# NUStatBioinfo/DegNorm

Hardware: AMD Instinct MI355X
Metric: genes/sec (20k genes x 10 samples, 5 iters) (higher is better)
Workload: dtype f64

## Files before the change

### degnorm_amd/csrc/dn_kernels.hpp

```cpp
#pragma once
#include <hip/hip_runtime.h>
#include <stddef.h>
#include <stdint.h>
#include <type_traits>
#include "dn_reduce.hpp"
#include "dn_dpp_ops.hpp"

#ifdef DN_MARKS
#define DN_MARK(name) asm volatile("; DN_MARK " name)
#else
#define DN_MARK(name)
#endif

namespace dn {

constexpr int TRACE_LEN = 48;
constexpr int MAX_BINS = 64;
constexpr int P_MAX = 64;
constexpr int P_WIDE_MAX = 256;

enum { EXIT_LOW_COV = 0, EXIT_ZERO_SAMPLE = 1, EXIT_MEDIAN = 2, EXIT_NO_LOOP = 3,
       EXIT_REFINED = 4, EXIT_REFINE_FALLBACK = 5, EXIT_NOT_FOUND_FALLBACK = 6 };
enum { LOOP_NATURAL = 0, LOOP_PERFECT = 1, LOOP_VALUE_ERROR = 2, LOOP_ZERO_ROWSUM = 3, LOOP_MIN_BINS = 4,
       LOOP_NOT_ENTERED = 5 };
// ... 656 lines not shown
    y = lds_row_dot<P>(Gr, uv);
    theta = wave_allsum(ul * y);
    return capped ? maxs + 1 : (steps < maxs ? steps + 1 : maxs);
}

constexpr double WARM_START_MIN_COMPONENT = 1e-7;
template <int P, bool DPP = (P <= 16)> struct Solver;
template <int P> struct Solver<P, true> {
    EigStateD<P> st;
    __device__ __forceinline__ double iterate_of_row() const { return st.vl; }
    static __device__ __forceinline__ int row_of_lane() { return lane_id() & 15; }
    static __device__ __forceinline__ double bcast_component(double t, int i) { return bcast_lane<P>(t, i); }
    __device__ __forceinline__ void cold(double tr, double (&u)[P]) { (void) u; eig_state_cold<P>(st, tr); }
    __device__ __forceinline__ void start_from(unsigned long long rows, double (&u)[P])
    {
        (void) u;
        const double u0 = 1.0 / sqrt((double) __builtin_popcountll(rows));
        st.vl = ((rows >> (lane_id() & 15)) & 1ull) ? u0 : 0.0;
        st.k0 = 0; st.rho2 = 1.0; st.q = 1.0; st.age = 0;
    }
    __device__ __forceinline__ void no_shift()
    {
        st.mu = 0.0;
    }
    __device__ __forceinline__ double shift() const { return st.mu; }
    __device__ __forceinline__ double scale() const { return st.sc; }
    static constexpr bool SHIFTED = true;
    static constexpr bool SQUARE = true;
    template <bool SQ = false>
    __device__ __forceinline__ int run(const double *tot, int zslot, double (&u)[P], double &theta, bool exact, int maxs, bool cold = false,
                                       const double *sq = nullptr)
    {
        return top_eig_dpp<P, false, SQ>(tot, zslot, u, theta, st, exact, cold, maxs, nullptr, sq);
    }
};
template <int P> struct Solver<P, false> {
    __device__ __forceinline__ void cold(double tr, double (&u)[P])
    {
        (void) tr;
        const double u0 = 1.0 / sqrt((double) P);
#pragma unroll
        for (int i = 0; i < P; i++) u[i] = u0;
    }
    __device__ __forceinline__ void start_from(unsigned long long rows, double (&u)[P])
    {
        const double u0 = 1.0 / sqrt((double) __builtin_popcountll(rows));
#pragma unroll
        for (int i = 0; i < P; i++) u[i] = ((rows >> i) & 1ull) ? u0 : 0.0;
    }
    __device__ __forceinline__ void no_shift() {}
    __device__ __forceinline__ double shift() const { return 0.0; }
    __device__ __forceinline__ double scale() const { return 1.0; }
    static constexpr bool SHIFTED = false;
    static constexpr bool SQUARE = false;
    template <bool SQ = false>
    __device__ __forceinline__ int run(const double *tot, int zslot, double (&u)[P], double &theta, bool exact, int maxs, bool cold = false,
                                       const double *sq = nullptr)
    { (void) zslot; (void) exact; (void) cold; (void) sq; return top_eig_rows<P>(tot, u, theta, maxs); }
};

__device__ __forceinline__ unsigned long long uniform_u64(unsigned long long x)
{
    const unsigned lo = __builtin_amdgcn_readfirstlane((unsigned) x), hi = __builtin_amdgcn_readfirstlane((unsigned) (x >> 32));
    return ((unsigned long long) hi << 32) | lo;
}

__device__ __forceinline__ unsigned long long gram_component(const double *tot, int seed, int nrows)
{
    const int lane = lane_id();
    unsigned long long comp = 1ull << seed, frontier = comp;
    while (frontier) {
        const int i = __builtin_ctzll(frontier);
        frontier &= frontier - 1ull;
        const int j = lane < nrows ? lane : 0;
        const int a = i > j ? i : j, b = i > j ? j : i;
        const bool link = lane < nrows && j != i && tot[a * (a + 1) / 2 + b] > 0.0;
        const unsigned long long fresh = uniform_u64(__ballot(link)) & ~comp;
        comp |= fresh;
        frontier |= fresh;
    }
    return comp;
}

template <int P>
__device__ __forceinline__ int solve_by_blocks(Solver<P> &solver, const double *tot, int zslot, double (&u)[P], double &theta,
                                               int maxs, int nrows = P)
{
    unsigned long long todo = nrows >= 64 ? ~0ull : ((1ull << nrows) - 1ull);
    const Solver<P> entry = solver;
    Solver<P> best = solver;
    double bu[P], bth = -1.0;
#pragma unroll
    for (int i = 0; i < P; i++) bu[i] = 0.0;
    int steps = 0;
    bool capped = false;
    while (todo) {
        const unsigned long long comp = gram_component(tot, __builtin_ctzll(todo), nrows);
        todo &= ~comp;
        Solver<P> s = entry;
        double uu[P], th = 0.0;
#pragma unroll
        for (int i = 0; i < P; i++) uu[i] = 0.0;
        s.start_from(comp, uu);
        const int r = s.run(tot, zslot, uu, th, true, maxs);
        steps += r < maxs ? r : maxs;
        capped = capped || r > maxs;
        if (th > bth) {
            bth = th;
            best = s;
#pragma unroll
            for (int i = 0; i < P; i++) bu[i] = uu[i];
        }
    }
    solver = best;
    solver.no_shift();
#pragma unroll
    for (int i = 0; i < P; i++) u[i] = bu[i];
    theta = bth > 0.0 ? bth : 0.0;
    return capped ? maxs + 1 : (steps < maxs ? steps : maxs);
}

typedef double gram_t;

template <int P, int LO, int CNT, typename T>
__device__ __forceinline__ void gram_add_range(T (&G)[CNT], const double (&a)[P])
{
    T b[P];
#pragma unroll
    for (int i = 0; i < P; i++) b[i] = (T) a[i];
#pragma unroll
    for (int i = 0; i < P; i++)
#pragma unroll
        for (int j = 0; j <= i; j++) {
            constexpr int dummy = 0; (void) dummy;
            const int idx = i * (i + 1) / 2 + j;
            if (idx >= LO && idx < LO + CNT) G[idx - LO] = fma(b[i], b[j], G[idx - LO]);
        }
}

template <int P, int LO, int CNT, typename T>
__device__ __forceinline__ void gram_set_range(T (&G)[CNT], const double (&a)[P])
{
    T b[P];
#pragma unroll
    for (int i = 0; i < P; i++) b[i] = (T) a[i];
#pragma unroll
    for (int i = 0; i < P; i++)
#pragma unroll
        for (int j = 0; j <= i; j++) {
            const int idx = i * (i + 1) / 2 + j;
            if (idx >= LO && idx < LO + CNT) G[idx - LO] = b[i] * b[j];
        }
}

template <int P, typename T>
__device__ __forceinline__ void gram_add(T (&G)[P * (P + 1) / 2], const double (&a)[P])
{
    T b[P];
#pragma unroll
    for (int i = 0; i < P; i++) b[i] = (T) a[i];
#pragma unroll
    for (int i = 0; i < P; i++)
#pragma unroll
        for (int j = 0; j <= i; j++) G[i * (i + 1) / 2 + j] = fma(b[i], b[j], G[i * (i + 1) / 2 + j]);
}

template <int P> __device__ __forceinline__ double vmax(const double (&v)[P])
{ double m = v[0];
#pragma unroll
  for (int i = 1; i < P; i++) m = v[i] > m ? v[i] : m; return m; }
template <int P> __device__ __forceinline__ double vmin(const double (&v)[P])
{ double m = v[0];
#pragma unroll
  for (int i = 1; i < P; i++) m = v[i] < m ? v[i] : m; return m; }

template <int P> __device__ __forceinline__ int fix_k(double (&K)[P])
{
    double mn = INFINITY;
#pragma unroll
    for (int i = 0; i < P; i++) { K[i] = fabs(K[i]); if (K[i] >= 1e-5 && K[i] < mn) mn = K[i]; }
    if (mn == INFINITY) return ST_EMPTY_MIN;
#pragma unroll
    for (int i = 0; i < P; i++) if (K[i] < 1e-5) K[i] = mn;
    return ST_OK;
}

template <int P> __device__ __forceinline__ double median_of(const double (&v)[P])
{
    double lo = 0.0, hi = 0.0;
#pragma unroll
    for (int i = 0; i < P; i++) {
        int less = 0, eq = 0;
#pragma unroll
        for (int j = 0; j < P; j++) { less += v[j] < v[i]; eq += v[j] == v[i]; }
        const int r_lo = (P - 1) / 2, r_hi = P / 2;
        if (less <= r_lo && r_lo < less + eq) lo = v[i];
        if (less <= r_hi && r_hi < less + eq) hi = v[i];
    }
    return 0.5 * (lo + hi);
}

template <int P>
struct GeneState {
    double sumF[P];
    double rho[P];
    double K[P];
    double us[P];
    double rho_fb[P];
    double sig0;
    double inv[P];
    double scl[P];
    double u[P];
    double theta;
    double sums[2 * P + 1];
    int32_t steps;
    int32_t status;
    int32_t max_steps;
#ifdef DN_STAMP
    long long stamp[8];
#else
    long long stamp[6];
#endif
};

#ifdef DN_P
__shared__ Smem<DN_P, DN_NT> g_sm_u[DN_UNITS];
__shared__ GeneState<DN_P> g_gs_u[DN_UNITS];
extern __shared__ __attribute__((aligned(16))) double g_lam[];
#define g_sm g_sm_u[DN_UNIT]
#define g_gs g_gs_u[DN_UNIT]
typedef const float __attribute__((address_space(1))) *gF_cptr;
typedef double __attribute__((address_space(1))) *gdouble_ptr;

template <int P>
__device__ __forceinline__ void col_update(const double (&f)[P], double (&a)[P], const double (&u)[P], const double (&ur)[P], double c)
{
    double s0 = 0.0, s1 = 0.0;
#pragma unroll
    for (int i = 0; i + 1 < P; i += 2) { s0 = fma(u[i], a[i], s0); s1 = fma(u[i + 1], a[i + 1], s1); }
    if (P & 1) s0 = fma(u[P - 1], a[P - 1], s0);
    const double s = s0 + s1;
#pragma unroll
    for (int i = 0; i < P; i++) {
        const double res = fma(ur[i], s, -f[i]);
        a[i] = fmax(fma(-c, res, a[i]), f[i]);
    }
}

template <int P>
__device__ __forceinline__ void col_update_lds(const float (&x)[P], const double *invp, double (&a)[P], const double *uv, double c)
{
    double s0 = 0.0, s1 = 0.0;
#pragma unroll
    for (int i = 0; i + 1 < P; i += 2) {
        const double2 u2 = *reinterpret_cast<const double2 *>(uv + i);
        s0 = fma(u2.x, a[i], s0); s1 = fma(u2.y, a[i + 1], s1);
    }
    if (P & 1) s0 = fma(uv[P - 1], a[P - 1], s0);
    const double s = s0 + s1;
#pragma unroll
    for (int i = 0; i < P; i++) {
        const double fi = (double) x[i] * invp[i];
        const double res = fma(uv[i], s, -fi);
        a[i] = fmax(fma(-c, res, a[i]), fi);
    }
}

template <int P>
__device__ __forceinline__ void col_final(const double (&f)[P], const double (&a)[P], const double (&u)[P], bool first,
                                          double (&acc)[2 * P + 1], double &s_out, double &r_out)
{
    double s = 0.0;
#pragma unroll
    for (int i = 0; i < P; i++) s = fma(u[i], a[i], s);
    acc[0] += s;
    double rmax = 0.0;
#pragma unroll
    for (int i = 0; i < P; i++) {
        const double ke = u[i] * s;
        acc[1 + i] += ke < f[i] ? f[i] : ke;
        acc[1 + P + i] += f[i];
        double d = ke - f[i];
        if (!first) d = d < 0.0 ? 0.0 : d;
        const double r = d * rcp_newton(f[i] + 1.0);
        const double r2 = r * r;
        rmax = r2 > rmax ? r2 : rmax;
    }
    s_out = s; r_out = rmax;
}

template <int PS>
__device__ __forceinline__ void lds_col_read(const double *col, double (&a)[PS])
{
#pragma unroll
    for (int i = 0; i < PS; i += 2) { const double2 v = *reinterpret_cast<const double2 *>(col + i); a[i] = v.x; a[i + 1] = v.y; }
}
template <int PS>
__device__ __forceinline__ void lds_col_write(double *col, const double (&a)[PS])
{
#pragma unroll
    for (int i = 0; i < PS; i += 2) *reinterpret_cast<double2 *>(col + i) = make_double2(a[i], a[i + 1]);
}

typedef float dn_f4 __attribute__((ext_vector_type(4)));
typedef float dn_f2 __attribute__((ext_vector_type(2)));
typedef dn_f4 dn_f4u __attribute__((aligned(4)));
typedef dn_f2 dn_f2u __attribute__((aligned(4)));
typedef const dn_f4u __attribute__((address_space(1))) *gF4_cptr;
typedef const dn_f2u __attribute__((address_space(1))) *gF2_cptr;

template <int P>
__device__ __forceinline__ void load_x(gF_cptr Fb, int k, float (&x)[P])
{
    gF_cptr col = Fb + (size_t) k * P;
#pragma unroll
    for (int i = 0; i + 4 <= P; i += 4) {
        const dn_f4 v = *(gF4_cptr) (col + i);
        x[i] = v.x; x[i + 1] = v.y; x[i + 2] = v.z; x[i + 3] = v.w;
    }
    if constexpr ((P & 3) >= 2) {
        const dn_f2 v = *(gF2_cptr) (col + (P & ~3));
        x[P & ~3] = v.x; x[(P & ~3) + 1] = v.y;
    }
    if constexpr (P & 1) x[P - 1] = col[P - 1];
}

template <int P>
__device__ __forceinline__ void load_f(gF_cptr Fb, int k, const double (&inv)[P], double (&f)[P])
{
    float x[P];
    load_x<P>(Fb, k, x);
#pragma unroll
    for (int i = 0; i < P; i++) f[i] = (double) x[i] * inv[i];
}

template <int P, bool RAW>
__device__ __forceinline__ void pass_counts(const float (&x)[P], const double (&inv)[P], double (&f)[P])
{
#pragma unroll
    for (int i = 0; i < P; i++) f[i] = RAW ? (double) x[i] : (double) x[i] * inv[i];
}

typedef double dn_d2 __attribute__((ext_vector_type(2)));
typedef dn_d2 __attribute__((address_space(1))) *gd2_ptr;
template <int P> constexpr int spill_mid() { return (P + (P & 1)) / 4; }
template <int P>
__device__ __forceinline__ gd2_ptr spill_col(gdouble_ptr Lg, int k)
{
    constexpr int PS = P + (P & 1);
    gd2_ptr col = (gd2_ptr) (Lg + ((size_t) (k >> 6) * (64 * PS) + (size_t) (k & 63) * 2)) + spill_mid<P>() * 64;
    asm volatile("" : "+v"(col));
    return col;
}
template <int P>
__device__ __forceinline__ void spill_col_read(gd2_ptr col, double (&a)[P])
{
#pragma unroll
    for (int q = 0; q < (P + 1) / 2; q++) {
        const dn_d2 v = col[(q - spill_mid<P>()) * 64];
        a[2 * q] = v.x;
        if (2 * q + 1 < P) a[2 * q + 1] = v.y;
    }
}
template <int P>
__device__ __forceinline__ void spill_col_write(gd2_ptr col, const double (&a)[P])
{
#pragma unroll
    for (int q = 0; q < (P + 1) / 2; q++) col[(q - spill_mid<P>()) * 64] = dn_d2{a[2 * q], 2 * q + 1 < P ? a[2 * q + 1 < P ? 2 * q + 1 : 2 * q] : 0.0};
}

template <int P, int NT>
__device__ __forceinline__ int mg_core(gF_cptr Fb, gdouble_ptr Lg, double *lam, int n, int nL, int T,
                                       double (&u)[P], double &theta, int &steps, int maxs, bool &noconv)
{
    constexpr int W = NT / 64;
    constexpr int NG = P * (P + 1) / 2;
    constexpr int PS = P + (P & 1);
    constexpr int TR = Smem<P, NT>::MG_TR, STR = Smem<P, NT>::MG_STR;
    constexpr int NTILE = TR * (TR + 1) / 2;
    Smem<P, NT> &sm = g_sm;
    const int tid = DN_TIDX, lane = lane_id(), w = wave_id();
    const int nLe = (n < nL) ? n : nL;
    double *stage = &sm.stage[w * 16 * STR];
    double *uv = &sm.eigv[w * 128], *vv = uv + 64;
    const double *invp = g_gs.inv;
    for (int e = lane; e < 16 * STR; e += 64) stage[e] = 0.0;
    uv[lane] = lane < P ? 1.0 / sqrt((double) P) : 0.0;
    vv[lane] = 0.0;
    wave_fence();
    const int oi = lane & 15, okq = lane >> 4;
    dn_double4 acc[NTILE];

    auto feed = [&](const double (&a)[PS], bool valid) {
#pragma unroll
        for (int cq = 0; cq < 4; cq++) {
            if ((lane >> 4) == cq) {
                double *dst = stage + (lane & 15) * STR;
#pragma unroll
                for (int i = 0; i < PS; i += 2) *reinterpret_cast<double2 *>(dst + i) = make_double2(valid ? a[i] : 0.0, valid ? a[i + 1] : 0.0);
            }
            wave_fence();
#pragma unroll
            for (int g = 0; g < 4; g++) {
                double x[TR];
#pragma unroll
                for (int tr = 0; tr < TR; tr++) x[tr] = stage[(4 * g + okq) * STR + 16 * tr + oi];
                int tix = 0;
#pragma unroll
                for (int t1 = 0; t1 < TR; t1++)
#pragma unroll
                    for (int t2 = 0; t2 <= t1; t2++, tix++)
                        acc[tix] = __builtin_amdgcn_mfma_f64_16x16x4f64(x[t1], x[t2], acc[tix], 0, 0, 0);
            }
            wave_fence();
        }
    };

    const double c = 1.0 / sqrt((double) T);
    auto pass = [&](bool cold, int t) {
#pragma unroll
        for (int i = 0; i < NTILE; i++) acc[i] = dn_double4{0.0, 0.0, 0.0, 0.0};
        const int wb = w * 64;
        const int steps_l = wb < nLe ? (nLe - wb + NT - 1) / NT : 0;
        const int steps_s = nL + wb < n ? (n - nL - wb + NT - 1) / NT : 0;
#pragma clang loop unroll(disable)
        for (int j = 0; j < steps_l; j++) {
            const int k = tid + j * NT;
            const bool valid = k < nLe;
            double a[PS];
#pragma unroll
            for (int i = 0; i < PS; i++) a[i] = 0.0;
            if (valid) {
                float xr[P];
                load_x<P>(Fb, k, xr);
                if (cold) {
#pragma unroll
                    for (int i = 0; i < P; i++) a[i] = (double) xr[i] * invp[i];
                } else {
                    double al[PS], aa[P];
                    lds_col_read<PS>(lam + (size_t) k * PS, al);
#pragma unroll
                    for (int i = 0; i < P; i++) aa[i] = al[i];
                    col_update_lds<P>(xr, invp, aa, uv, c);
#pragma unroll
                    for (int i = 0; i < P; i++) a[i] = aa[i];
                }
                lds_col_write<PS>(lam + (size_t) k * PS, a);
            }
            feed(a, valid);
        }
#pragma clang loop unroll(disable)
        for (int j = 0; j < steps_s; j++) {
            const int k = nL + tid + j * NT;
            const bool valid = k < n;
            double a[PS];
#pragma unroll
            for (int i = 0; i < PS; i++) a[i] = 0.0;
            if (valid) {
                float xr[P];
                double aa[P];
                load_x<P>(Fb, k, xr);
                const gd2_ptr col = spill_col<P>(Lg, k);
                if (cold) {
#pragma unroll
                    for (int i = 0; i < P; i++) aa[i] = (double) xr[i] * invp[i];
                } else {
                    spill_col_read<P>(col, aa);
                    col_update_lds<P>(xr, invp, aa, uv, c);
                }
                spill_col_write<P>(col, aa);
#pragma unroll
                for (int i = 0; i < P; i++) a[i] = aa[i];
            }
            feed(a, valid);
        }
        {
            double *dst = (W > 1) ? sm.xw[w] : sm.tot;
            int tix = 0;
#pragma unroll
            for (int t1 = 0; t1 < TR; t1++)
#pragma unroll
                for (int t2 = 0; t2 <= t1; t2++, tix++)
#pragma unroll
                    for (int r = 0; r < 4; r++) {
                        const int row = 16 * t1 + okq + 4 * r, col = 16 * t2 + oi;
                        if (row < P && col <= row) dst[row * (row + 1) / 2 + col] = acc[tix][r];
                    }
        }
        if constexpr (W > 1) {
            dn_sync();
            for (int e = tid; e < NG; e += NT) {
                double tsum = sm.xw[0][e];
#pragma unroll
                for (int ww = 1; ww < W; ww++) tsum += sm.xw[ww][e];
                sm.tot[e] = tsum;
            }
        }
        dn_sync();
    };

    pass(true, 0);
    {
        const double tr = wave_allsum(lane < P ? sm.tot[lane * (lane + 1) / 2 + lane] : 0.0);
        if (!(tr > 0.0)) return ST_ARPACK;
    }
    { const int r = top_eig_rows_lds<P>(sm.tot, uv, vv, theta, maxs); steps += r; noconv = noconv || r > maxs; }
    bool cold_every_solve;
    {
        double um = lane < P ? uv[lane] : 1.0;
#pragma unroll
        for (int o = 32; o >= 1; o >>= 1) um = fmin(um, __shfl_xor(um, o));
        cold_every_solve = __builtin_amdgcn_readfirstlane((int) (um < WARM_START_MIN_COMPONENT)) != 0;
    }
#pragma clang loop unroll(disable)
    for (int t = 0; t < T; t++) {
        pass(false, t);
        int r;
        if (!cold_every_solve) r = top_eig_rows_lds<P>(sm.tot, uv, vv, theta, maxs);
        else {
            unsigned long long todo = P >= 64 ? ~0ull : ((1ull << P) - 1ull);
            double bul = 0.0, bth = -1.0;
            int sum = 0;
            bool capped = false;
            while (todo) {
                const unsigned long long comp = gram_component(sm.tot, __builtin_ctzll(todo), P);
                todo &= ~comp;
                wave_fence();
                uv[lane] = ((comp >> lane) & 1ull) ? 1.0 / sqrt((double) __builtin_popcountll(comp)) : 0.0;
                wave_fence();
                double th = 0.0;
                const int rr = top_eig_rows_lds<P>(sm.tot, uv, vv, th, maxs);
                sum += rr < maxs ? rr : maxs;
                capped = capped || rr > maxs;
                const double ul = uv[lane];
                if (th > bth) { bth = th; bul = ul; }
            }
            wave_fence();
            uv[lane] = bul;
            wave_fence();
            theta = bth > 0.0 ? bth : 0.0;
            r = capped ? maxs + 1 : (sum < maxs ? sum : maxs);
        }
        steps += r; noconv = noconv || r > maxs;
    }
    bcast_rows<P>(lane < P ? uv[lane] : 0.0, u);
    return ST_OK;
}

#ifndef DN_RT_MAX_COLS
#define DN_RT_MAX_COLS 12
#endif
#ifndef DN_RT_MAX_P
#define DN_RT_MAX_P 12
#endif
#ifndef DN_RT_MIN_P
#define DN_RT_MIN_P 2
#endif
#if defined(DN_P) && DN_P >= DN_RT_MIN_P && DN_P <= DN_RT_MAX_P
#define DN_REG_TIER 1
#define DN_KERNEL_WAVES 2
#define DN_RT_CLAIM() asm volatile("" ::: "a255")
#else
#define DN_REG_TIER 0
#define DN_KERNEL_WAVES 1
#define DN_RT_CLAIM()
#endif
#define DN_RAW_MAX_P 12
template <int P> constexpr bool raw_units() { return DN_REG_TIER != 0 && P <= DN_RAW_MAX_P && P < DN_MG_MIN_P; }

template <int IDX> __device__ __forceinline__ int agpr_get1();
template <int IDX> __device__ __forceinline__ void agpr_put1(int v);
#define DN_AGPR_ACCESSORS(N)                                                                                              \
    template <> __device__ __forceinline__ int agpr_get1<N>() { int v; asm volatile("v_accvgpr_read_b32 %0, a" #N : "=v"(v)); return v; } \
    template <> __device__ __forceinline__ void agpr_put1<N>(int v) { asm volatile("v_accvgpr_write_b32 a" #N ", %0" : : "v"(v)); }
#define DN_AGPR_REGS(X) \
    X(0) X(1) X(2) X(3) X(4) X(5) X(6) X(7) X(8) X(9) X(10) X(11) X(12) X(13) X(14) X(15) \
    X(16) X(17) X(18) X(19) X(20) X(21) X(22) X(23) X(24) X(25) X(26) X(27) X(28) X(29) X(30) X(31) \
    X(32) X(33) X(34) X(35) X(36) X(37) X(38) X(39) X(40) X(41) X(42) X(43) X(44) X(45) X(46) X(47) \
    X(48) X(49) X(50) X(51) X(52) X(53) X(54) X(55) X(56) X(57) X(58) X(59) X(60) X(61) X(62) X(63) \
    X(64) X(65) X(66) X(67) X(68) X(69) X(70) X(71) X(72) X(73) X(74) X(75) X(76) X(77) X(78) X(79) \
    X(80) X(81) X(82) X(83) X(84) X(85) X(86) X(87) X(88) X(89) X(90) X(91) X(92) X(93) X(94) X(95) \
    X(96) X(97) X(98) X(99) X(100) X(101) X(102) X(103) X(104) X(105) X(106) X(107) X(108) X(109) X(110) X(111) \
    X(112) X(113) X(114) X(115) X(116) X(117) X(118) X(119) X(120) X(121) X(122) X(123) X(124) X(125) X(126) X(127) \
    X(128) X(129) X(130) X(131) X(132) X(133) X(134) X(135) X(136) X(137) X(138) X(139) X(140) X(141) X(142) X(143) \
    X(144) X(145) X(146) X(147) X(148) X(149) X(150) X(151) X(152) X(153) X(154) X(155) X(156) X(157) X(158) X(159) \
    X(160) X(161) X(162) X(163) X(164) X(165) X(166) X(167) X(168) X(169) X(170) X(171) X(172) X(173) X(174) X(175) \
    X(176) X(177) X(178) X(179) X(180) X(181) X(182) X(183) X(184) X(185) X(186) X(187) X(188) X(189) X(190) X(191) \
    X(192) X(193) X(194) X(195) X(196) X(197) X(198) X(199) X(200) X(201) X(202) X(203) X(204) X(205) X(206) X(207) \
    X(208) X(209) X(210) X(211) X(212) X(213) X(214) X(215) X(216) X(217) X(218) X(219) X(220) X(221) X(222) X(223) \
    X(224) X(225) X(226) X(227) X(228) X(229) X(230) X(231) X(232) X(233) X(234) X(235) X(236) X(237) X(238) X(239) \
    X(240) X(241) X(242) X(243) X(244) X(245) X(246) X(247) X(248) X(249) X(250) X(251) X(252) X(253) X(254) X(255)
DN_AGPR_REGS(DN_AGPR_ACCESSORS)
#undef DN_AGPR_ACCESSORS
#undef DN_AGPR_REGS
template <int IDX> __device__ __forceinline__ double agpr_get()
{
    const int lo = agpr_get1<IDX>(), hi = agpr_get1<IDX + 1>();
    return __hiloint2double(hi, lo);
}
template <int IDX> __device__ __forceinline__ void agpr_put(double v)
{
    agpr_put1<IDX>(__double2loint(v));
    agpr_put1<IDX + 1>(__double2hiint(v));
}

template <int P, int BASE> __device__ __forceinline__ void rt_read(double (&a)[P])
{
    static_for<0, P>([&](auto ic) { constexpr int I = decltype(ic)::value; a[I] = agpr_get<BASE + 2 * I>(); });
}
template <int P, int BASE> __device__ __forceinline__ void rt_write(const double (&a)[P])
{
    static_for<0, P>([&](auto ic) { constexpr int I = decltype(ic)::value; agpr_put<BASE + 2 * I>(a[I]); });
}
template <int P, int BASE> __device__ __forceinline__ void rt_read_counts(double (&xd)[P])
{
    static_for<0, (P + 1) / 2>([&](auto jc) {
        constexpr int J = decltype(jc)::value;
        const unsigned w = (unsigned) agpr_get1<BASE + J>();
        xd[2 * J] = (double) (w & 0xffffu);
        if constexpr (2 * J + 1 < P) xd[2 * J + 1] = (double) (w >> 16);
    });
}
template <int P, int BASE> __device__ __forceinline__ void rt_write_counts(const float (&x)[P])
{
    static_for<0, (P + 1) / 2>([&](auto jc) {
        constexpr int J = decltype(jc)::value;
        unsigned w = (unsigned) x[2 * J];
        if constexpr (2 * J + 1 < P) w |= ((unsigned) x[2 * J + 1]) << 16;
        agpr_put1<BASE + J>((int) w);
    });
}
template <int P, bool X16> constexpr int rt_col_regs() { return 2 * P + (X16 ? (P + 1) / 2 : 0); }
template <int P, bool X16> constexpr int rt_cols()
{
    return (P >= DN_RT_MIN_P && P <= DN_RT_MAX_P) ? (256 / rt_col_regs<P, X16>() < DN_RT_MAX_COLS ? 256 / rt_col_regs<P, X16>() : DN_RT_MAX_COLS) : 0;
}
template <int P> constexpr int rt_regs_used()
{
    return rt_cols<P, true>() * rt_col_regs<P, true>() > rt_cols<P, false>() * rt_col_regs<P, false>()
               ? rt_cols<P, true>() * rt_col_regs<P, true>() : rt_cols<P, false>() * rt_col_regs<P, false>();
}
constexpr int RT_BATCH = 48;
#define DN_RT_SAVE_IDX(r) ((size_t) (r) * NT + DN_TIDX)
template <int N, int NT> __device__ __forceinline__ void rt_save(int *save, int need)
{
    static_for<0, (N + RT_BATCH - 1) / RT_BATCH>([&](auto bc) {
        constexpr int B = decltype(bc)::value * RT_BATCH;
        constexpr int CNT = (N - B) < RT_BATCH ? (N - B) : RT_BATCH;
        if (B < need) {
            int v[CNT];
            static_for<0, CNT>([&](auto ic) { constexpr int I = decltype(ic)::value; v[I] = agpr_get1<B + I>(); });
#pragma unroll
            for (int i = 0; i < CNT; i++) save[DN_RT_SAVE_IDX(B + i)] = v[i];
            asm volatile("" ::: "memory");
        }
    });
}
template <int N, int NT> __device__ __forceinline__ void rt_restore(const int *save, int need)
{
    static_for<0, (N + RT_BATCH - 1) / RT_BATCH>([&](auto bc) {
        constexpr int B = decltype(bc)::value * RT_BATCH;
        constexpr int CNT = (N - B) < RT_BATCH ? (N - B) : RT_BATCH;
        if (B < need) {
            int v[CNT];
#pragma unroll
            for (int i = 0; i < CNT; i++) v[i] = save[DN_RT_SAVE_IDX(B + i)];
            static_for<0, CNT>([&](auto ic) { constexpr int I = decltype(ic)::value; agpr_put1<B + I>(v[I]); });
            asm volatile("" ::: "memory");
        }
    });
}
template <int R, int RT, typename F>
__device__ __forceinline__ void partial_rounds(int nr, F &&column)
{
    if constexpr (R < RT) {
        if (R == 0 || R < nr) {
            column(std::integral_constant<int, R>{});
            __builtin_amdgcn_sched_barrier(0);
            partial_rounds<R + 1, RT>(nr, column);
        }
    }
}
template <int P, int NT> constexpr size_t rt_save_bytes() { return (size_t) rt_regs_used<P>() * 4 * NT; }

template <int P, int NT, bool X16, bool FULL = false, bool ONCHIP = false, bool SAFE = false>
__device__ __forceinline__ void nmf_body(const float *Fb_, double *Lg_, double *rs_, double *sv_,
                                         int n, int S, int nL, int T, int first_i)
{
    Smem<P, NT> &sm = g_sm;
    double *lam = g_lam + (DN_UNITS > 1 ? (size_t) DN_UNIT * (size_t) nL * (P + (P & 1)) : 0);
    gF_cptr Fb = (gF_cptr) uniform_ptr(Fb_);
    gdouble_ptr Lg = (gdouble_ptr) uniform_ptr(Lg_);
    gdouble_ptr rs = (gdouble_ptr) uniform_ptr(rs_);
    gdouble_ptr sv = (gdouble_ptr) uniform_ptr(sv_);
    n = __builtin_amdgcn_readfirstlane(n);
    S = __builtin_amdgcn_readfirstlane(S);
    nL = __builtin_amdgcn_readfirstlane(nL);
    T = __builtin_amdgcn_readfirstlane(T);
    const bool first = __builtin_amdgcn_readfirstlane(first_i) != 0;
    double inv[P], u[P], theta = 0.0;
    int steps = 0;
    const int maxs = __builtin_amdgcn_readfirstlane(g_gs.max_steps);
    bool noconv = false;
#pragma unroll
    for (int i = 0; i < P; i++) inv[i] = uniform(g_gs.inv[i]);
    long long stamp[4] = {0, 0, 0, 0};
#ifdef DN_STAMP
#define DN_T0() const long long t0_ = __builtin_amdgcn_s_memtime()
#define DN_T1(slot) stamp[slot] += __builtin_amdgcn_s_memtime() - t0_
#else
#define DN_T0()
#define DN_T1(slot) (void) stamp
#endif
    constexpr int NG = P * (P + 1) / 2;
    constexpr int CH_MAX = P <= 15 ? 120 : 90;
    constexpr int SW = (NG + CH_MAX - 1) / CH_MAX;
    constexpr int CH = (NG + SW - 1) / SW;
    constexpr int PS = P + (P & 1);
    const int tid = DN_TIDX;
    constexpr int RT = DN_REG_TIER ? rt_cols<P, X16>() : 0;
    constexpr int CS = rt_col_regs<P, X16>();
    constexpr int NR = RT * NT;
    constexpr bool RAW = raw_units<P>();
    double ud[P], ur[P];
    const int nLe = (n < NR + nL) ? n : NR + nL;
    const int kS0 = NR + nL;
    if constexpr (P >= DN_MG_MIN_P) {
        const int st = mg_core<P, NT>(Fb, Lg, lam, n, nL, T, u, theta, steps, maxs, noconv);
        if (st != ST_OK) { if (tid == 0) g_gs.status = st; dn_sync(); return; }
    } else {
    gram_t G[CH];

#ifdef DN_STAMP
    const long long t_cold0 = __builtin_amdgcn_s_memtime();
#endif
#pragma unroll
    for (int i = 0; i < CH; i++) G[i] = 0.0;
    {
        float xq[P];
        if (tid < n) load_x<P>(Fb, tid, xq);
#pragma clang loop unroll(disable)
        for (int k = tid; k < n; k += NT) {
            double f[P];
#pragma unroll
            for (int i = 0; i < P; i++) f[i] = (double) xq[i] * inv[i];
            load_x<P>(Fb, k + NT < n ? k + NT : k, xq);
            gram_add_range<P, 0, CH>(G, f);
        }
    }
    block_sum_lds<CH, P, NT, gram_t>(G, sm);
    static_for<1, SW>([&](auto qc) {
        constexpr int Q = decltype(qc)::value;
        constexpr int NQ = (NG - Q * CH) < CH ? (NG - Q * CH) : CH;
        gram_t Gq[NQ];
#pragma unroll
        for (int i = 0; i < NQ; i++) Gq[i] = 0.0;
#pragma clang loop unroll(disable)
        for (int k = tid; k < n; k += NT) {
            double f[P];
            load_f<P>(Fb, k, inv, f);
            gram_add_range<P, Q * CH, NQ>(Gq, f);
        }
        block_sum_lds<NQ, P, NT, gram_t, false, Q * CH>(Gq, g_sm);
    });
    {
        double tr = 0.0;
#pragma unroll
        for (int i = 0; i < P; i++) tr += sm.tot[i * (i + 1) / 2 + i];
        if (!(tr > 0.0)) { if (tid == 0) g_gs.status = ST_ARPACK; dn_sync(); return; }
    }
    Solver<P> solver;
    {
        double tr = 0.0;
#pragma unroll
        for (int i = 0; i < P; i++) tr += sm.tot[i * (i + 1) / 2 + i];
        solver.cold(tr, u);
    }
    {
        const int r = SAFE ? solve_by_blocks<P>(solver, sm.tot, Smem<P, NT>::ZSLOT, u, theta, maxs)
                           : solver.run(sm.tot, Smem<P, NT>::ZSLOT, u, theta, T == 0, maxs, true);
        steps += r; noconv = noconv || r > maxs;
    }
    const double c = 1.0 / sqrt((double) T);
    auto pass_u = [&]() {
        if constexpr (RAW) {
            const int k = Solver<P>::row_of_lane() < P ? Solver<P>::row_of_lane() : P - 1;
            const double vt = solver.iterate_of_row() * g_gs.inv[k], vh = solver.iterate_of_row() * g_gs.scl[k];
#pragma unroll
            for (int i = 0; i < P; i++) { ud[i] = Solver<P>::bcast_component(vt, i); ur[i] = Solver<P>::bcast_component(vh, i); }
        } else {
#pragma unroll
            for (int i = 0; i < P; i++) { u[i] = uniform(u[i]); ud[i] = u[i]; ur[i] = u[i]; }
        }
    };
    pass_u();

    constexpr bool PART = RT > 0 && X16 && !FULL;
    const int nr = (n + NT - 1) / NT;
    static_for<0, RT>([&](auto rc) {
        constexpr int R = decltype(rc)::value;
        const int k = tid + R * NT;
        if constexpr (PART) {
            if (R < nr) {
                float xf[P];
                double f[P];
#pragma unroll
                for (int i = 0; i < P; i++) xf[i] = 0.0f;
                if (k < n) load_x<P>(Fb, k, xf);
                pass_counts<P, RAW>(xf, inv, f);
                rt_write<P, CS * R>(f);
                rt_write_counts<P, CS * R + 2 * P>(xf);
            }
        } else if (k < n) {
            float xf[P];
            double f[P];
            load_x<P>(Fb, k, xf);
            pass_counts<P, RAW>(xf, inv, f);
            rt_write<P, CS * R>(f);
            if constexpr (X16) rt_write_counts<P, CS * R + 2 * P>(xf);
        }
    });
    for (int k = NR + tid; k < nLe; k += NT) {
        double f[P], a[PS];
        { float xf[P]; load_x<P>(Fb, k, xf); pass_counts<P, RAW>(xf, inv, f); }
#pragma unroll
        for (int i = 0; i < PS; i++) a[i] = i < P ? f[i] : 0.0;
        lds_col_write<PS>(lam + (size_t) (k - NR) * PS, a);
    }
    if constexpr (!ONCHIP) {
        for (int k = kS0 + tid; k < n; k += NT) {
            double f[P];
            { float xf[P]; load_x<P>(Fb, k, xf); pass_counts<P, RAW>(xf, inv, f); }
            spill_col_write<P>(spill_col<P>(Lg, k), f);
        }
    }
#ifdef DN_STAMP
    stamp[3] += __builtin_amdgcn_s_memtime() - t_cold0;
#endif
    constexpr bool G0 = FULL && ONCHIP && SW == 1;
    constexpr bool SQ = Solver<P>::SQUARE && SW == 1 && !SAFE;
#pragma clang loop unroll(disable)
    for (int t = 0; t < T; t++) {
        DN_MARK("iter_begin");
        auto gram_zero = [&]() {
#pragma unroll
            for (int i = 0; i < CH; i++) G[i] = 0.0;
        };
        if constexpr (!G0 && !PART) gram_zero();
        DN_MARK("zeroed");
        { DN_T0();
        const int dir = (t & 1) ? -1 : 1;

        auto reg_tier = [&](auto start) {
            if constexpr (RT > 0 && X16) {
                auto column = [&](auto rc) {
                    constexpr int R = decltype(rc)::value;
                    double f[P], a[P];
                    rt_read_counts<P, CS * R + 2 * P>(f);
                    if constexpr (!RAW) {
#pragma unroll
                        for (int i = 0; i < P; i++) f[i] *= inv[i];
                    }
                    rt_read<P, CS * R>(a);
                    col_update<P>(f, a, ud, ur, c);
                    if constexpr (decltype(start)::value && R == 0) gram_set_range<P, 0, CH>(G, a); else gram_add_range<P, 0, CH>(G, a);
                    rt_write<P, CS * R>(a);
                };
                if constexpr (FULL) {
                    static_for<0, RT>([&](auto rc) { column(rc); __builtin_amdgcn_sched_barrier(0); });
                } else {
                    partial_rounds<0, RT>(nr, column);
                }
            } else if constexpr (RT > 0) {
                float xq[P];
                if (tid < n) load_x<P>(Fb, tid, xq);
                static_for<0, RT>([&](auto rc) {
                    constexpr int R = decltype(rc)::value;
                    const int k = tid + R * NT;
                    if (k < n) {
                        double f[P], a[P];
                        pass_counts<P, RAW>(xq, inv, f);
                        if constexpr (R + 1 < RT) load_x<P>(Fb, k + NT < n ? k + NT : k, xq);
                        rt_read<P, CS * R>(a);
                        col_update<P>(f, a, ud, ur, c);
                        gram_add_range<P, 0, CH>(G, a);
                        rt_write<P, CS * R>(a);
                    }
                });
            }
        };
        auto lds_tier = [&]() {
            const int first = NR + tid;
            const int cnt = first < nLe ? (nLe - first + NT - 1) / NT : 0;
            const int step = dir * NT;
            int k = dir > 0 ? first : first + (cnt - 1) * NT;
            float xq[P];
            if (cnt > 0) load_x<P>(Fb, k, xq);
#pragma clang loop unroll(disable)
            for (int j = 0; j < cnt; j++, k += step) {
                double f[P], a[PS];
                lds_col_read<PS>(lam + (size_t) (k - NR) * PS, a);
                pass_counts<P, RAW>(xq, inv, f);
                load_x<P>(Fb, j + 1 < cnt ? k + step : k, xq);
                double aa[P];
#pragma unroll
                for (int i = 0; i < P; i++) aa[i] = a[i];
                col_update<P>(f, aa, ud, ur, c);
                gram_add_range<P, 0, CH>(G, aa);
#pragma unroll
                for (int i = 0; i < P; i++) a[i] = aa[i];
                lds_col_write<PS>(lam + (size_t) (k - NR) * PS, a);
            }
        };
        auto spill_tier = [&]() {
            if constexpr (ONCHIP) return;
            int tq = tid;
            asm volatile("" : "+v"(tq));
            const int first = kS0 + tq;
            if (first >= n) return;
            const int step = dir * NT;
            const int last = first + (n - 1 - first) / NT * NT;
            int k = dir > 0 ? first : last;
            const int kend = dir > 0 ? last : first;
            float xn[P];
            double an[P];
            load_x<P>(Fb, k, xn);
            spill_col_read<P>(spill_col<P>(Lg, k), an);
            bool more;
#pragma clang loop unroll(disable)
            do {
                double f[P], a[P];
                pass_counts<P, RAW>(xn, inv, f);
#pragma unroll
                for (int i = 0; i < P; i++) a[i] = an[i];
                const int kn = dir > 0 ? min(k + step, kend) : max(k + step, kend);
                load_x<P>(Fb, kn, xn);
                spill_col_read<P>(spill_col<P>(Lg, kn), an);
                col_update<P>(f, a, ud, ur, c);
                gram_add_range<P, 0, CH>(G, a);
                spill_col_write<P>(spill_col<P>(Lg, k), a);
                more = k != kend;
                k += step;
            } while (more);
        };
#if defined(DN_STAMP) && defined(DN_EXP_TIER)
#define DN_TIER(id, call) do { if (DN_EXP_TIER == id) { const long long tt_ = __builtin_amdgcn_s_memtime(); call; stamp[0] += __builtin_amdgcn_s_memtime() - tt_; } else { call; } } while (0)
#else
#define DN_TIER(id, call) call
#endif
        if constexpr (PART) {
            const bool mem = n > NR;
            if (dir > 0) { DN_MARK("reg_tier"); DN_TIER(1, reg_tier(std::true_type{})); if (mem) { DN_MARK("lds_tier"); DN_TIER(2, lds_tier()); DN_MARK("spill_tier"); DN_TIER(3, spill_tier()); } }
            else { gram_zero(); if (mem) { DN_MARK("spill_tier_b"); DN_TIER(3, spill_tier()); DN_MARK("lds_tier_b"); DN_TIER(2, lds_tier()); } DN_MARK("reg_tier_b"); DN_TIER(1, reg_tier(std::false_type{})); }
        }
        else if constexpr (G0) { DN_MARK("reg_tier"); DN_TIER(1, reg_tier(std::true_type{})); DN_MARK("lds_tier"); DN_TIER(2, lds_tier()); }
        else if (dir > 0) { DN_MARK("reg_tier"); DN_TIER(1, reg_tier(std::false_type{})); DN_MARK("lds_tier"); DN_TIER(2, lds_tier()); DN_MARK("spill_tier"); DN_TIER(3, spill_tier()); }
        else { DN_MARK("spill_tier_b"); DN_TIER(3, spill_tier()); DN_MARK("lds_tier_b"); DN_TIER(2, lds_tier()); DN_MARK("reg_tier_b"); DN_TIER(1, reg_tier(std::false_type{})); }
        DN_MARK("pass_end");
#if !(defined(DN_STAMP) && defined(DN_EXP_TIER))
        DN_T1(0);
#endif
        }
        { DN_T0(); block_sum_lds<CH, P, NT, gram_t, Solver<P>::SHIFTED, 0, RAW, SQ>(G, sm, solver.shift(), solver.scale(), t & 1); DN_T1(1); }
        DN_MARK("reduced");
        static_for<1, SW>([&](auto qc) {
            constexpr int Q = decltype(qc)::value;
            constexpr int NQ = (NG - Q * CH) < CH ? (NG - Q * CH) : CH;
            gram_t Gq[NQ];
#pragma unroll
            for (int i = 0; i < NQ; i++) Gq[i] = 0.0;
            static_assert(SW == 1 || RT == 0, "the later sweeps do not read the register tier");
#pragma clang loop unroll(disable)
            for (int k = NR + tid; k < nLe; k += NT) {
                double a[PS], aa[P];
                lds_col_read<PS>(lam + (size_t) (k - NR) * PS, a);
#pragma unroll
                for (int i = 0; i < P; i++) aa[i] = a[i];
                gram_add_range<P, Q * CH, NQ>(Gq, aa);
            }
#pragma clang loop unroll(disable)
            for (int k = kS0 + tid; k < n; k += NT) {
                double aa[P];
                spill_col_read<P>(spill_col<P>(Lg, k), aa);
                gram_add_range<P, Q * CH, NQ>(Gq, aa);
            }
            block_sum_lds<NQ, P, NT, gram_t, Solver<P>::SHIFTED, Q * CH>(Gq, g_sm, solver.shift());
        });
        { DN_T0();
        double u_unused[P];
        double (&us_)[P] = RAW ? u_unused : u;
        const int r = SAFE ? solve_by_blocks<P>(solver, sm.tot, Smem<P, NT>::ZSLOT, us_, theta, maxs)
                           : solver.template run<SQ>(sm.tot, Smem<P, NT>::ZSLOT, us_, theta, t == T - 1, maxs, false,
                                                     sm.sq + wave_id() * Smem<P, NT>::SQ_LEN);
        steps += r; noconv = noconv || r > maxs;
        pass_u();
        DN_MARK("solved");
        DN_T1(2);
        }
    }
    if constexpr (SQ && NT > 64) dn_sync();
    if constexpr (RAW) {
#pragma unroll
        for (int i = 0; i < P; i++) u[i] = Solver<P>::bcast_component(solver.iterate_of_row(), i);
    }
    }

#ifdef DN_STAMP
    const long long t_fin0 = __builtin_amdgcn_s_memtime();
#endif
    double invf[P];
#pragma unroll
    for (int i = 0; i < P; i++) invf[i] = RAW ? uniform(g_gs.inv[i]) : inv[i];
    double acc[2 * P + 1];
#pragma unroll
    for (int i = 0; i < 2 * P + 1; i++) acc[i] = 0.0;
    auto fin = [&](int k, const double (&f)[P], const double (&l_)[P]) {
        double s, r, l0[P];
#pragma unroll
        for (int i = 0; i < P; i++) l0[i] = RAW ? l_[i] * invf[i] : l_[i];
        col_final<P>(f, l0, u, first, acc, s, r);
        rs[k] = r;
        if (first) sv[k] = s;
    };
    static_for<0, RT>([&](auto rc) {
        constexpr int R = decltype(rc)::value;
        const int k = tid + R * NT;
        if (k < n) {
            double f[P], l[P];
            if constexpr (X16) {
                rt_read_counts<P, CS * R + 2 * P>(f);
#pragma unroll
                for (int i = 0; i < P; i++) f[i] *= invf[i];
            } else load_f<P>(Fb, k, invf, f);
            rt_read<P, CS * R>(l);
            fin(k, f, l);
        }
    });
    float xqf[P];
    if (NR + tid < n) load_x<P>(Fb, NR + tid, xqf);
#pragma clang loop unroll(disable)
    for (int k = NR + tid; k < n; k += NT) {
        double f[P], l[P];
#pragma unroll
        for (int i = 0; i < P; i++) f[i] = (double) xqf[i] * invf[i];
        load_x<P>(Fb, k + NT < n ? k + NT : k, xqf);
        if (k < nLe) {
            double al[PS];
            lds_col_read<PS>(lam + (size_t) (k - NR) * PS, al);
#pragma unroll
            for (int i = 0; i < P; i++) l[i] = al[i];
        } else spill_col_read<P>(spill_col<P>(Lg, k), l);
        fin(k, f, l);
    }
    block_sum_lds<2 * P + 1, P, NT, double>(acc, sm);
    for (int e = tid; e < 2 * P + 1; e += NT) g_gs.sums[e] = sm.tot[e];
    if (tid == 0) {
#pragma unroll
        for (int i = 0; i < P; i++) g_gs.u[i] = u[i];
        g_gs.theta = theta;
        g_gs.steps += steps;
        g_gs.status = noconv ? ST_NO_CONVERGENCE : ST_OK;
#ifdef DN_STAMP
        g_gs.stamp[0] += stamp[0]; g_gs.stamp[1] += stamp[1]; g_gs.stamp[2] += stamp[2];
        g_gs.stamp[4] += __builtin_amdgcn_s_memtime() - t_fin0; g_gs.stamp[5] += stamp[3];
        if constexpr (RT > 0 && X16 && !FULL) { g_gs.stamp[6] += stamp[0]; g_gs.stamp[7] += (long long) T * ((n + NT - 1) / NT); }
#endif
    }
    dn_sync();
}

template <int P, int NT, bool SAFE = false>
__device__ __attribute__((noinline)) void nmf_call(const float *Fb_, double *Lg_, double *rs_, double *sv_, double *rtsave_,
                                                   int n, int S, int nL, int T, int first_i, int x16_i)
{
    constexpr int NSAVE = DN_REG_TIER ? rt_regs_used<P>() : 0;
    int *rtsave = reinterpret_cast<int *>(uniform_ptr(rtsave_));
#ifdef DN_STAMP
    const long long t_call0 = __builtin_amdgcn_s_memtime();
#endif
    const int n_u = __builtin_amdgcn_readfirstlane(n);
    const int need = DN_REG_TIER ? ((n_u + NT - 1) / NT) * rt_col_regs<P, true>() : 0;
    rt_save<NSAVE, NT>(rtsave, need);
    if constexpr (SAFE) {
        nmf_body<P, NT, false, false, false, true>(Fb_, Lg_, rs_, sv_, n, S, nL, T, first_i);
    } else if (DN_REG_TIER && __builtin_amdgcn_readfirstlane(x16_i) != 0) {
        constexpr bool X = DN_REG_TIER != 0;
        const int nL_u = __builtin_amdgcn_readfirstlane(nL);
        if (X && n_u >= rt_cols<P, X>() * NT && n_u <= rt_cols<P, X>() * NT + nL_u)
            nmf_body<P, NT, X, X, X>(Fb_, Lg_, rs_, sv_, n, S, nL, T, first_i);
        else if (X && n_u >= rt_cols<P, X>() * NT) nmf_body<P, NT, X, X>(Fb_, Lg_, rs_, sv_, n, S, nL, T, first_i);
        else nmf_body<P, NT, X, false>(Fb_, Lg_, rs_, sv_, n, S, nL, T, first_i);
    } else nmf_body<P, NT, false>(Fb_, Lg_, rs_, sv_, n, S, nL, T, first_i);
    rt_restore<NSAVE, NT>(rtsave, need);
#ifdef DN_STAMP
    if (DN_TIDX == 0) g_gs.stamp[3] += __builtin_amdgcn_s_memtime() - t_call0;
#endif
}


template <int P> __device__ __forceinline__ double lds_max(const double *v)
{ double m = v[0];
#pragma unroll
  for (int i = 1; i < P; i++) { const double t = v[i]; m = t > m ? t : m; } return m; }
template <int P> __device__ __forceinline__ double lds_min(const double *v)
{ double m = v[0];
#pragma unroll
  for (int i = 1; i < P; i++) { const double t = v[i]; m = t < m ? t : m; } return m; }

template <int P, int NT>
__global__ __launch_bounds__(NT * DN_UNITS, DN_KERNEL_WAVES) void k_baseline(IterArgs A)
{
    constexpr int W = NT / 64;
    Smem<P, NT> &sm = g_sm;
    GeneState<P> &gs = g_gs;
    const int tid = DN_TIDX, lane = lane_id(), w = wave_id();
    const int S = A.S;
    const int nL = A.lds_cols;
    char *slot = A.ws + ((size_t) blockIdx.x * DN_UNITS + DN_UNIT) * A.slot_bytes;
    float *Fs = reinterpret_cast<float *>(slot);
    float *Fb = Fs + (size_t) P * S;
    double *Lg = reinterpret_cast<double *>(Fb + (size_t) P * S);
    double *sv = Lg + (size_t) (P + (P & 1)) * S;
    double *rs = sv + S;
    double *rtsave = rs + 2 * (size_t) S;
    DN_RT_CLAIM();
    if (tid < P) { gs.inv[tid] = A.inv_scale[tid]; gs.scl[tid] = 1.0 / A.inv_scale[tid]; }
    if (tid == 0) gs.max_steps = A.max_steps > 0 ? A.max_steps : EIG_MAX_STEPS_DEFAULT;
    if constexpr (P <= 16) { for (int t = tid; t < W * Smem<P, NT>::SQ_LEN; t += NT) sm.sq[t] = 0.0; }
    for (int t = tid; t < Smem<P, NT>::NX; t += NT) {
        bool diag = false;
        int ra = 0, rb = 0;
#pragma unroll
        for (int i = 0; i < P; i++) {
            diag = diag || (t == i * (i + 1) / 2 + i);
            if (t >= i * (i + 1) / 2) { ra = i; rb = t - i * (i + 1) / 2; }
        }
        if constexpr (P <= 16) sm.sqi[t] = (t < P * (P + 1) / 2) ? (ra * Smem<P, NT>::SQ_STR + rb) | ((rb * Smem<P, NT>::SQ_STR + ra) << 16) : 0;
        if constexpr (raw_units<P>())
            sm.dsel[t] = (t < P * (P + 1) / 2) ? (diag ? -1.0 : 1.0) * A.inv_scale[ra] * A.inv_scale[rb < P ? rb : 0] : 0.0;
        else sm.dsel[t] = diag ? 1.0 : 0.0;
        if (t == Smem<P, NT>::ZSLOT) sm.tot[t] = 0.0;
    }

    for (;;) {
        if (tid == 0) sm.gene = atomicAdd(A.counter, 1);
        dn_sync();
        const int q = sm.gene;
        dn_sync();
        if (q >= A.n_genes) break;
        const int g = A.order[q];
        const int L = A.glen[g];
        const float *x = A.cov + A.goff[g];

        int n0 = 0, n_calls = 0, n_drops = 0, exit_code = EXIT_LOW_COV, loop_reason = LOOP_NOT_ENTERED;
        int status = ST_OK, flag = 0, emode = EM_INPUT;
        long long sum_cols = 0;
#ifdef DN_STAMP
        const long long t_gene0 = __builtin_amdgcn_s_memtime();
        long long t_ret = 0, t_book = 0;
#endif
        int32_t *tr = A.trace + (size_t) g * TRACE_LEN;
        if (tid < P) { gs.rho[tid] = 0.0; gs.K[tid] = 0.0; gs.us[tid] = 0.0; }
        if (tid == 0) { gs.steps = 0; gs.stamp[0] = gs.stamp[1] = gs.stamp[2] = gs.stamp[3] = gs.stamp[4] = gs.stamp[5] = 0; }
#ifdef DN_STAMP
        if (tid == 0) gs.stamp[6] = gs.stamp[7] = 0;
#endif

        double thr;
        int x16;
        {
            const float *rmx = A.rowmax + (size_t) g * P;
            double gmax = (double) rmx[0] / A.scale[0];
#pragma unroll
            for (int i = 1; i < P; i++) { const double v = (double) rmx[i] / A.scale[i]; gmax = v > gmax ? v : gmax; }
            thr = 0.1 * gmax;
            x16 = A.x16[g];
        }

        const int rate = A.rate;
        const long long ds0 = (rate > 1 && A.ds_start) ? A.ds_start[g] : -1;
        const int M = ds0 >= 0 ? (ds0 < L ? (int) ((L - 1 - ds0) / rate) + 1 : 0) : L;
        const int seg = ((M + W - 1) / W + 63) & ~63;
        const int jb = w * seg, je = (jb + seg < M) ? jb + seg : M;

        {
            double sumF[P];
#pragma unroll
            for (int i = 0; i < P; i++) sumF[i] = 0.0;
            int base = 0;
            for (int pass = 0; pass < 2; pass++) {
                int run = 0;
                for (int c = jb; c < je; c += 64) {
                    const int m = c + lane;
                    bool hi = false;
                    float xv[P];
                    double f[P];
                    if (m < je) {
                        const long long j = ds0 >= 0 ? ds0 + (long long) m * rate : (long long) m;
                        double cm = 0.0;
#pragma unroll
                        for (int i = 0; i < P; i++) { xv[i] = x[(size_t) i * L + j]; f[i] = (double) xv[i] / A.scale[i]; cm = f[i] > cm ? f[i] : cm; }
                        hi = cm > thr;
                    }
                    const unsigned long long mask = __ballot(hi);
                    if (pass == 1 && hi) {
                        const int pos = base + run + __popcll(mask & ((1ull << lane) - 1ull));
#pragma unroll
                        for (int i = 0; i < P; i++) {
                            Fs[(size_t) i * S + pos] = xv[i];
                            Fb[(size_t) pos * P + i] = xv[i];
                            sumF[i] += f[i];
                        }
                    }
                    run += __popcll(mask);
                }
// ... 389 lines not shown
```

Measured before the change: 15630.

## Software-pipeline LDS column reads in lds_tier with inline-asm ds_read_b128

Rewrites the LDS tier loop so the next column's LDS read is issued with inline-asm ds_read_b128 right after the current column is stored. An explicit lgkmcnt wait is deferred until the data is needed, so LDS latency overlaps the Gram accumulation and the global count prefetch. Compiler barriers pin instruction order and keep NR in a scalar register. The cost is manual waitcnt management and a store-then-reload ordering that relies on LDS in-order semantics; columns past P are written as zeros.

```diff
diff --git a/degnorm_amd/csrc/dn_kernels.hpp b/degnorm_amd/csrc/dn_kernels.hpp
--- a/degnorm_amd/csrc/dn_kernels.hpp
+++ b/degnorm_amd/csrc/dn_kernels.hpp
@@ -982,6 +982,54 @@
     for (int i = 0; i < PS; i += 2) *reinterpret_cast<double2 *>(col + i) = make_double2(a[i], a[i + 1]);
 }
 
+typedef double dn_d2 __attribute__((ext_vector_type(2)));
+__device__ __forceinline__ unsigned lds_byte_addr(const double *p)
+{
+    return (unsigned) (size_t) (const __attribute__((address_space(3))) double *) p;
+}
+#define DN_LDS_PLANES(X) X(0) X(1) X(2) X(3) X(4) X(5) X(6) X(7) X(8) X(9) X(10) X(11)
+template <int PS>
+__device__ __forceinline__ void lds_col_request(unsigned addr, dn_d2 (&v)[PS / 2])
+{
+    static_assert(PS % 2 == 0 && PS >= 2 && PS <= 24, "one statement per double2 of the column");
+#define DN_LDS_READ(Q) \
+    if constexpr (Q < PS / 2) asm volatile("ds_read_b128 %0, %1 offset:%2" : "=v"(v[Q < PS / 2 ? Q : 0]) : "v"(addr), "i"(Q * 16));
+    DN_LDS_PLANES(DN_LDS_READ)
+#undef DN_LDS_READ
+}
+template <int PS>
+__device__ __forceinline__ void lds_col_store(unsigned addr, const dn_d2 (&v)[PS / 2])
+{
+    static_assert(PS % 2 == 0 && PS >= 2 && PS <= 24, "one statement per double2 of the column");
+#define DN_LDS_WRITE(Q) \
+    if constexpr (Q < PS / 2) asm volatile("ds_write_b128 %0, %1 offset:%2" : : "v"(addr), "v"(v[Q < PS / 2 ? Q : 0]), "i"(Q * 16));
+    DN_LDS_PLANES(DN_LDS_WRITE)
+#undef DN_LDS_WRITE
+}
+#undef DN_LDS_PLANES
+template <int PS>
+__device__ __forceinline__ void lds_col_wait(dn_d2 (&v)[PS / 2])
+{
+    constexpr int N = PS / 2;
+    static_assert(PS % 2 == 0 && N >= 1 && N <= 12, "one operand per double2 of the column");
+#define DN_V(Q) "+v"(v[Q < N ? Q : 0])
+#define DN_WAIT(...) asm volatile("s_waitcnt lgkmcnt(0)" : __VA_ARGS__)
+    if constexpr (N == 1) DN_WAIT(DN_V(0));
+    else if constexpr (N == 2) DN_WAIT(DN_V(0), DN_V(1));
+    else if constexpr (N == 3) DN_WAIT(DN_V(0), DN_V(1), DN_V(2));
+    else if constexpr (N == 4) DN_WAIT(DN_V(0), DN_V(1), DN_V(2), DN_V(3));
+    else if constexpr (N == 5) DN_WAIT(DN_V(0), DN_V(1), DN_V(2), DN_V(3), DN_V(4));
+    else if constexpr (N == 6) DN_WAIT(DN_V(0), DN_V(1), DN_V(2), DN_V(3), DN_V(4), DN_V(5));
+    else if constexpr (N == 7) DN_WAIT(DN_V(0), DN_V(1), DN_V(2), DN_V(3), DN_V(4), DN_V(5), DN_V(6));
+    else if constexpr (N == 8) DN_WAIT(DN_V(0), DN_V(1), DN_V(2), DN_V(3), DN_V(4), DN_V(5), DN_V(6), DN_V(7));
+    else if constexpr (N == 9) DN_WAIT(DN_V(0), DN_V(1), DN_V(2), DN_V(3), DN_V(4), DN_V(5), DN_V(6), DN_V(7), DN_V(8));
+    else if constexpr (N == 10) DN_WAIT(DN_V(0), DN_V(1), DN_V(2), DN_V(3), DN_V(4), DN_V(5), DN_V(6), DN_V(7), DN_V(8), DN_V(9));
+    else if constexpr (N == 11) DN_WAIT(DN_V(0), DN_V(1), DN_V(2), DN_V(3), DN_V(4), DN_V(5), DN_V(6), DN_V(7), DN_V(8), DN_V(9), DN_V(10));
+    else DN_WAIT(DN_V(0), DN_V(1), DN_V(2), DN_V(3), DN_V(4), DN_V(5), DN_V(6), DN_V(7), DN_V(8), DN_V(9), DN_V(10), DN_V(11));
+#undef DN_WAIT
+#undef DN_V
+}
+
 typedef float dn_f4 __attribute__((ext_vector_type(4)));
 typedef float dn_f2 __attribute__((ext_vector_type(2)));
 typedef dn_f4 dn_f4u __attribute__((aligned(4)));
@@ -1021,7 +1069,6 @@
     for (int i = 0; i < P; i++) f[i] = RAW ? (double) x[i] : (double) x[i] * inv[i];
 }
 
-typedef double dn_d2 __attribute__((ext_vector_type(2)));
 typedef dn_d2 __attribute__((address_space(1))) *gd2_ptr;
 template <int P> constexpr int spill_mid() { return (P + (P & 1)) / 4; }
 template <int P>
@@ -1570,27 +1617,46 @@
             }
         };
         auto lds_tier = [&]() {
-            const int first = NR + tid;
+            int nr0 = NR;
+            asm volatile("" : "+s"(nr0));
+            const int first = nr0 + tid;
             const int cnt = first < nLe ? (nLe - first + NT - 1) / NT : 0;
             const int step = dir * NT;
-            int k = dir > 0 ? first : first + (cnt - 1) * NT;
+            int k = cnt > 0 ? (dir > 0 ? first : first + (cnt - 1) * NT) : NR;
+            unsigned la = lds_byte_addr(lam) + (unsigned) (k - NR) * (unsigned) (PS * 8);
+            const int lstep = step * (PS * 8);
             float xq[P];
-            if (cnt > 0) load_x<P>(Fb, k, xq);
+            dn_d2 v[PS / 2];
+            load_x<P>(Fb, min(k, n - 1), xq);
+            lds_col_request<PS>(la, v);
 #pragma clang loop unroll(disable)
-            for (int j = 0; j < cnt; j++, k += step) {
-                double f[P], a[PS];
-                lds_col_read<PS>(lam + (size_t) (k - NR) * PS, a);
+            for (int j = 0; j < cnt; j++) {
+                double f[P];
                 pass_counts<P, RAW>(xq, inv, f);
-                load_x<P>(Fb, j + 1 < cnt ? k + step : k, xq);
+                const bool more = j + 1 < cnt;
+                int kn = k + step;
+                unsigned ln = la + (unsigned) lstep;
+                asm volatile("" : "+v"(kn), "+v"(ln));
+                kn = more ? kn : k;
+#pragma unroll
+                for (int i = 0; i < P; i++) asm volatile("" : "+v"(kn) : "v"(f[i]));
+                load_x<P>(Fb, kn, xq);
+                lds_col_wait<PS>(v);
                 double aa[P];
 #pragma unroll
-                for (int i = 0; i < P; i++) aa[i] = a[i];
+                for (int i = 0; i < P; i++) aa[i] = v[i / 2][i & 1];
                 col_update<P>(f, aa, ud, ur, c);
+#pragma unroll
+                for (int i = 0; i < PS; i++) v[i / 2][i & 1] = i < P ? aa[i] : 0.0;
+                lds_col_store<PS>(la, v);
+                la = more ? ln : la;
+                lds_col_request<PS>(la, v);
+#pragma unroll
+                for (int i = 0; i < P; i++) asm volatile("" : "+v"(aa[i]));
                 gram_add_range<P, 0, CH>(G, aa);
-#pragma unroll
-                for (int i = 0; i < P; i++) a[i] = aa[i];
-                lds_col_write<PS>(lam + (size_t) (k - NR) * PS, a);
+                k = kn;
             }
+            lds_col_wait<PS>(v);
         };
         auto spill_tier = [&]() {
             if constexpr (ONCHIP) return;
```

Result: no change. 15610 (-0.2%).
